# AzureLeon1/DiffSpectra

Hardware: AMD Instinct MI355X
Metric: molecules/sec, 1000-step QM9S all-spectra sampling (partial run) (higher is better)
Workload: dtype f32 (GEMMs as split-fp16 x3 MFMA with fp32 accumulate; fp32-level accuracy, parity gates unchanged)

## Files before the change

diffspectra_amd/csrc/ds_device.h:

```cpp
#pragma once
#include <hip/hip_runtime.h>
#include <stdint.h>

typedef float f32x16 __attribute__((ext_vector_type(16)));
typedef float f32x2 __attribute__((ext_vector_type(2)));
typedef _Float16 h4 __attribute__((ext_vector_type(4)));
typedef _Float16 h8 __attribute__((ext_vector_type(8)));
typedef float f32x4 __attribute__((ext_vector_type(4)));

#define DS_LDP 4

__device__ __forceinline__ float ds_silu(float x) { return __fdividef(x, 1.0f + __expf(-x)); }
__device__ __forceinline__ float ds_tanh(float x) {
  const float e = __builtin_amdgcn_exp2f(x * 2.8853900817779268f);
  return fmaf(-2.0f, __builtin_amdgcn_rcpf(e + 1.0f), 1.0f);
}
__device__ __forceinline__ f32x2 ds_tanh2_prescaled(f32x2 t) {
  f32x2 e;
  e.x = __builtin_amdgcn_exp2f(t.x); e.y = __builtin_amdgcn_exp2f(t.y);
  const f32x2 d = e + 1.0f;
  f32x2 r;
  r.x = __builtin_amdgcn_rcpf(d.x); r.y = __builtin_amdgcn_rcpf(d.y);
  return r * -2.0f + 1.0f;
}
// ... 327 lines not shown
#pragma unroll
  for (int m = 0; m < MT; ++m) {
    xa[m][0] = *reinterpret_cast<const h8*>(xr + m * 32 * ldh);
    xa[m][1] = *reinterpret_cast<const h8*>(xr + m * 32 * ldh + K_tile);
  }
#define DS_MMA_(ACC, WV, XV) ACC = TRANS ? __builtin_amdgcn_mfma_f32_32x32x16_f16(WV, XV, ACC, 0, 0, 0) : __builtin_amdgcn_mfma_f32_32x32x16_f16(XV, WV, ACC, 0, 0, 0)
#pragma unroll
  for (int i = 0; i < NKB; ++i) {
    const int in = i + 1 < NKB ? i + 1 : i;
    h8 xn[MT][2];
#pragma unroll
    for (int m = 0; m < MT; ++m) {
      xn[m][0] = *reinterpret_cast<const h8*>(xr + m * 32 * ldh + in * 16);
      xn[m][1] = *reinterpret_cast<const h8*>(xr + m * 32 * ldh + K_tile + in * 16);
    }
    __builtin_amdgcn_sched_barrier(0);
    const h8 a1 = ringA.w1[i % PF], a2 = ringA.w2[i % PF], b1 = ringB.w1[i % PF], b2 = ringB.w2[i % PF];
#pragma unroll
    for (int m = 0; m < MT; ++m) { DS_MMA_(loA[m], a1, xa[m][1]); DS_MMA_(loB[m], b1, xa[m][1]); }
#pragma unroll
    for (int m = 0; m < MT; ++m) { DS_MMA_(hiA[m], a1, xa[m][0]); DS_MMA_(hiB[m], b1, xa[m][0]); }
#pragma unroll
    for (int m = 0; m < MT; ++m) { DS_MMA_(loA[m], a2, xa[m][0]); DS_MMA_(loB[m], b2, xa[m][0]); }
    if (i + PF < NKB) {
      ringA.w1[i % PF] = wload_h(wsA, 0, kb0 + i + PF); ringA.w2[i % PF] = wload_h(wsA, 1, kb0 + i + PF);
      ringB.w1[i % PF] = wload_h(wsB, 0, kb0 + i + PF); ringB.w2[i % PF] = wload_h(wsB, 1, kb0 + i + PF);
    }
    __builtin_amdgcn_sched_barrier(0);
#pragma unroll
    for (int m = 0; m < MT; ++m) { xa[m][0] = xn[m][0]; xa[m][1] = xn[m][1]; }
  }
#undef DS_MMA_
}
template <int MT, bool TRANS, int NKB, int PF>
__device__ __forceinline__ void wave_mma_h_ring_t2(const _Float16* X, int K_tile, const WStreamH& wsA, const WStreamH& wsB, int kb0,
                                                   f32x16 (&hiA)[MT], f32x16 (&loA)[MT], f32x16 (&hiB)[MT], f32x16 (&loB)[MT], int xkb0 = 0) {
  WRingH<PF> ringA, ringB;
#pragma unroll
  for (int i = 0; i < PF; ++i) {
    ringA.w1[i] = wload_h(wsA, 0, kb0 + i); ringA.w2[i] = wload_h(wsA, 1, kb0 + i);
    ringB.w1[i] = wload_h(wsB, 0, kb0 + i); ringB.w2[i] = wload_h(wsB, 1, kb0 + i);
    __builtin_amdgcn_sched_barrier(0);
  }
  wave_mma_h_deep_t2<MT, TRANS, NKB, PF>(X, K_tile, wsA, wsB, ringA, ringB, kb0, hiA, loA, hiB, loB, xkb0);
}

template <int MT, bool TRANS, int NKB, int PF>
__device__ __forceinline__ void wave_mma_h_ring(const _Float16* X, int K_tile, const float* __restrict__ Wh, int N, int K, int col0,
                                                int kb0, f32x16 (&hi)[MT], f32x16 (&lo)[MT], int xkb0 = 0) {
  const WStreamH ws = wstream_h(Wh, N, K, col0);
  WRingH<PF> ring;
  wring_h<PF>(ring, ws, kb0);
  wave_mma_h_deep<MT, TRANS, NKB, PF>(X, K_tile, ws, ring, kb0, hi, lo, xkb0);
}
template <int MT>
__device__ __forceinline__ void split_finish(f32x16 (&hi)[MT], const f32x16 (&lo)[MT]) {
#pragma unroll
  for (int m = 0; m < MT; ++m)
#pragma unroll
    for (int i = 0; i < 16; ++i) hi[m][i] = fmaf(lo[m][i], 1.0f / 2048.0f, hi[m][i]);
}

template <int MT>
__device__ __forceinline__ void acc_zero(f32x16 (&acc)[MT]) {
#pragma unroll
  for (int m = 0; m < MT; ++m)
#pragma unroll
    for (int i = 0; i < 16; ++i) acc[m][i] = 0.0f;
}

template <int MT, class F>
__device__ __forceinline__ void acc_foreach(const f32x16 (&acc)[MT], int row_base, int col0, F f) {
  const int lane = threadIdx.x & 63, r = lane & 31, hh = lane >> 5;
#pragma unroll
  for (int m = 0; m < MT; ++m)
#pragma unroll
    for (int i = 0; i < 16; ++i) f(row_base + m * 32 + acc_row(i, hh), col0 + r, acc[m][i]);
}

struct RowStore {
  __amdgpu_buffer_rsrc_t rsrc;
  int voff;
};
template <int LD>
__device__ __forceinline__ RowStore row_store(float* dst) {
  const int lane = threadIdx.x & 63;
  const unsigned long long pw = reinterpret_cast<unsigned long long>(dst);
  const unsigned long long pu = (static_cast<unsigned long long>(__builtin_amdgcn_readfirstlane(static_cast<int>(pw >> 32))) << 32) |
                                static_cast<unsigned int>(__builtin_amdgcn_readfirstlane(static_cast<int>(pw)));
  RowStore s;
  s.rsrc = __builtin_amdgcn_make_buffer_rsrc(reinterpret_cast<float*>(pu), 0, 0x7fffffff, 0x00020000);
  s.voff = ((4 * (lane >> 5)) * LD + (lane & 31)) * 4;
  return s;
}
__device__ __forceinline__ void row_put(const RowStore& s, int row_byte_off, float v) {
  __builtin_amdgcn_raw_buffer_store_b32(__float_as_uint(v), s.rsrc, s.voff, row_byte_off, 0);
}
template <int MT, int LD, class F>
__device__ __forceinline__ void acc_store(const f32x16 (&acc)[MT], float* __restrict__ dst, int rows_valid, F f) {
  const int lane = threadIdx.x & 63, r = lane & 31, hh = lane >> 5;
  const RowStore st = row_store<LD>(dst);
  if (rows_valid >= 32 * MT) {
#pragma unroll
    for (int m = 0; m < MT; ++m)
#pragma unroll
      for (int i = 0; i < 16; ++i) row_put(st, (m * 32 + (i & 3) + 8 * (i >> 2)) * LD * 4, f(r, acc[m][i]));
  } else {
#pragma unroll
    for (int m = 0; m < MT; ++m)
#pragma unroll
      for (int i = 0; i < 16; ++i) {
        const int row = m * 32 + (i & 3) + 8 * (i >> 2);
        if (row + 4 * hh < rows_valid) row_put(st, row * LD * 4, f(r, acc[m][i]));
      }
  }
}

template <int MTOT, int MT>
__device__ __forceinline__ BFrag tile_first(const float* __restrict__ Wp, int Npad, int K, int nch) {
  constexpr int RG = MTOT / MT;
  const int wave = threadIdx.x >> 6;
  const int it = wave < nch * RG ? wave : 0;
  return bfrag_load(Wp, Npad, (it / RG) * 32, 0, K >> 3);
}

template <int MTOT, int MT, class G>
__device__ __forceinline__ void tile_gemm_blk(const float* X, int ldx, int K, const float* __restrict__ Wp, int Npad, int nch,
                                              G g, const BFrag* first = nullptr) {
  static_assert(MTOT % MT == 0, "row tiling");
// ... 30 lines not shown
```

diffspectra_amd/csrc/ds_forward.hip:

```cpp
#include <hip/hip_runtime.h>
#include <math.h>
#include <stdint.h>
#include <stdlib.h>

#include <atomic>
#include <mutex>
#include <utility>
#include <vector>

#include "../../include/diffspectra_hip.h"
#include "ds_device.h"
#include "ds_host.h"

#define ADAC DS_ADA_COLS
constexpr int DS_NODE_PF = 8;
constexpr int DS_NODE_PF2 = 4;
constexpr int DS_QKV_PF = 4;
constexpr int DS_TWO_STREAM_MAX_PAIRS = 400000;

#ifdef DS_STAMPS
#define DS_STAMP_INIT()                                                                                 \
  unsigned long long _sa[16] = {0, 0, 0, 0, 0, 0, 0, 0, 0, 0, 0, 0, 0, 0, 0, 0};                        \
  unsigned long long _t0 = __builtin_amdgcn_s_memtime()
#define DS_STAMP(i)                                                                                     \
// ... 6 lines not shown
  do {                                                                                                  \
    asm volatile("s_waitcnt vmcnt(0) lgkmcnt(0)" ::: "memory");                                         \
    DS_STAMP(i);                                                                                        \
  } while (0)
#define DS_STAMP_FLUSH(t)                                                                               \
  do {                                                                                                  \
    if (threadIdx.x == (t))                                                                             \
      for (int _i = 0; _i < 16; ++_i)                                                                   \
        if (_sa[_i]) atomicAdd(reinterpret_cast<unsigned long long*>(c.ws.flags + 16) + _i, _sa[_i]);   \
  } while (0)
#else
#define DS_STAMP_INIT()
#define DS_STAMP(i)
#define DS_STAMP_W(i)
#define DS_STAMP_FLUSH(t)
#endif

namespace {

using dst::clear;
using dst::record;
using dst::wait;

struct Ctx {
  ds_layout L;
  ds_workspace ws;
  const float* wbase;
  const int64_t* woff;
  float edge_th, cutoff;
};

__device__ __forceinline__ const float* BW(const Ctx& c, int blk, int slot) {
  return c.wbase + c.woff[blk * DS_W_BLOCK_SLOTS + slot];
}
__device__ __forceinline__ const float* GW(const Ctx& c, int slot) {
  return c.wbase + c.woff[DS_NBLOCKS * DS_W_BLOCK_SLOTS + slot];
}

__device__ __forceinline__ float rbf_feature(float x, int k, const float* __restrict__ mean, const float* __restrict__ stdv,
                                             const float* __restrict__ astd) {
  if (k == 0) return x;
  const float z = (x - mean[k - 1]) / stdv[k - 1];
  return expf(-0.5f * (z * z)) / astd[k - 1];
}

__global__ void k_time_feat(Ctx c, const float* __restrict__ noise_level) {
  const int b = blockIdx.x * blockDim.x + threadIdx.x;
  if (b >= c.L.B) return;
  const float* w = GW(c, DS_GW_SIN_W);
  const float x = noise_level[b];
  float* f = c.ws.tfeat + (size_t)b * 24;
  f[0] = x;
  for (int i = 0; i < 8; ++i) {
    const float fr = ((x * w[i]) * 2.0f) * 3.14159265358979323846f;
    f[1 + i] = sinf(fr);
    f[9 + i] = cosf(fr);
  }
  for (int i = 17; i < 24; ++i) f[i] = 0.0f;
}

__global__ void k_pair_flags(Ctx c, const float* __restrict__ cond_x, const float* __restrict__ cond_edge_x) {
  const int p = blockIdx.x * blockDim.x + threadIdx.x;
  const bool valid = p < c.L.Pp;
  int bits = 3;
  bool nonzero = false;
  if (valid && cond_x != nullptr) {
// ... 589 lines not shown
  const int Nn = c.L.Nn;
  {
    float4 v[16];
#pragma unroll
    for (int u = 0; u < 16; ++u) {
      const int idx = tid + u * 256, row = idx >> 6, k4 = idx & 63;
      v[u] = reinterpret_cast<const float4*>(c.ws.attn + (size_t)min(row0 + row, Nn - 1) * 256)[k4];
    }
#pragma unroll
    for (int u = 0; u < 16; ++u) {
      const int idx = tid + u * 256, row = idx >> 6, k4 = idx & 63;
      split_store4(&A1[row][0], 256, 4 * k4, row0 + row < Nn ? v[u] : make_float4(0, 0, 0, 0));
    }
  }
  __syncthreads();
  const int mt = wave >> 1, cc = wave & 1;
  if (row0 + mt * 32 >= Nn) return;
  f32x16 acc[1], lo[1];
  acc_zero<1>(acc);
  acc_zero<1>(lo);
  wave_mma_h_ring<1, false, 16, DS_NODE_PF>(&A1[mt * 32][0], 256, BW(c, blk, DS_BW_N2E_H), 64, 256, cc * 32, 0, acc, lo);
  split_finish<1>(acc, lo);
  acc_store<1, 64>(acc, c.ws.u + (size_t)(row0 + mt * 32) * 64 + cc * 32, Nn - row0 - mt * 32, [](int, float v) { return v; });
  (void)lane;
}

template <bool N2E>
__global__ __launch_bounds__(256, 2) void k_node_update(Ctx c, int blk) {
  ds_fp16_saturate();
  constexpr int T = 32, LDH = 2 * 256 + 8;
  __shared__ __attribute__((aligned(16))) _Float16 B1[T][LDH];
  __shared__ __attribute__((aligned(16))) _Float16 H2[T][LDH];
  __shared__ int rmol[T];
  const int tid = threadIdx.x, wave = tid >> 6, row0 = blockIdx.x * T;
  const int Nn = c.L.Nn;
  const float* ada = c.ws.ada;
  if (tid < T) rmol[tid] = (row0 + tid < Nn) ? c.L.node_mol[row0 + tid] : 0;
  __syncthreads();
  {
    const int lane = tid & 63, g = lane >> 4, j = lane & 15;
    float4 va[2][4], vh[2][4], vg[2][4], sh[2][4], sc[2][4];
#pragma unroll
    for (int ps = 0; ps < 2; ++ps) {
      const int row = 8 * wave + 4 * ps + g;
      const size_t gr = (size_t)min(row0 + row, Nn - 1);
      const float4* ad = reinterpret_cast<const float4*>(ada + (size_t)rmol[row] * ADAC + blk * DS_ADA_BLOCK_STRIDE + DS_ADA_NODE) + j;
      const float4* ap = reinterpret_cast<const float4*>(c.ws.attn + gr * 256) + j;
      const float4* hp = reinterpret_cast<const float4*>(c.ws.h + gr * 256) + j;
#pragma unroll
      for (int u = 0; u < 4; ++u) {
        va[ps][u] = ap[16 * u];
        vh[ps][u] = hp[16 * u];
        vg[ps][u] = ad[128 + 16 * u];
        sh[ps][u] = ad[192 + 16 * u];
        sc[ps][u] = ad[256 + 16 * u];
      }
    }
#pragma unroll
    for (int ps = 0; ps < 2; ++ps) {
      const int row = 8 * wave + 4 * ps + g;
      float4 r[4];
#pragma unroll
      for (int u = 0; u < 4; ++u) {
        if (row0 + row >= Nn) va[ps][u] = vh[ps][u] = make_float4(0, 0, 0, 0);
        if (N2E) split_store4(&B1[row][0], 256, 64 * u + 4 * j, va[ps][u]);
        r[u].x = vh[ps][u].x + vg[ps][u].x * va[ps][u].x; r[u].y = vh[ps][u].y + vg[ps][u].y * va[ps][u].y;
        r[u].z = vh[ps][u].z + vg[ps][u].z * va[ps][u].z; r[u].w = vh[ps][u].w + vg[ps][u].w * va[ps][u].w;
      }
      ln_mod_quad256(r, sh[ps], sc[ps]);
#pragma unroll
      for (int u = 0; u < 4; ++u) split_store4(&H2[row][0], 256, 64 * u + 4 * j, r[u]);
    }
  }
  __syncthreads();
  if (N2E) {
    if (wave < 2) {
      f32x16 acc[1], lo[1];
      acc_zero<1>(acc);
      acc_zero<1>(lo);
      wave_mma_h_ring<1, false, 16, DS_NODE_PF>(&B1[0][0], 256, BW(c, blk, DS_BW_N2E_H), 64, 256, wave * 32, 0, acc, lo);
      split_finish<1>(acc, lo);
      acc_store<1, 64>(acc, c.ws.u + (size_t)row0 * 64 + wave * 32, Nn - row0, [](int, float v) { return v; });
    }
    __syncthreads();
  }
  {
    const float* b1 = BW(c, blk, DS_BW_FF1_B);
    const float* W1 = BW(c, blk, DS_BW_FF1_H);
    const float* W2 = BW(c, blk, DS_BW_FF2_H);
    f32x16 acc2[2][1], lo2[2][1];
    acc_zero<1>(acc2[0]); acc_zero<1>(acc2[1]);
    acc_zero<1>(lo2[0]); acc_zero<1>(lo2[1]);
    const int mA = rmol[0], mB = rmol[min(T, Nn - row0) - 1];
    const float* gsec = ada + blk * DS_ADA_BLOCK_STRIDE + DS_ADA_NODE + 1280;
    float gAv[2], gBv[2], bbv[2];
#pragma unroll
    for (int cc = 0; cc < 2; ++cc) {
      const int col = (wave + 4 * cc) * 32 + (tid & 31);
      gAv[cc] = gsec[(size_t)mA * ADAC + col]; gBv[cc] = gsec[(size_t)mB * ADAC + col]; bbv[cc] = BW(c, blk, DS_BW_FF2_B)[col];
    }
    for (int half = 0; half < 2; ++half) {
      {
        asm volatile("" ::: "memory");
        const int hhf = (tid & 63) >> 5;
        f32x16 acc[2][1], lo[2][1];
#pragma unroll
        for (int cc = 0; cc < 2; ++cc) {
          const float bf = b1[half * 256 + (wave + 4 * cc) * 32 + (tid & 31)];
#pragma unroll
          for (int i = 0; i < 16; ++i) acc[cc][0][i] = bf;
          acc_zero<1>(lo[cc]);
        }
        wave_mma_h_ring_t2<1, false, 16, DS_NODE_PF2>(&H2[0][0], 256, wstream_h(W1, 512, 256, (half * 8 + wave) * 32),
                                                     wstream_h(W1, 512, 256, (half * 8 + wave + 4) * 32), 0, acc[0], lo[0], acc[1], lo[1]);
#pragma unroll
        for (int cc = 0; cc < 2; ++cc) {
          split_finish<1>(acc[cc], lo[cc]);
          const int colf = (wave + 4 * cc) * 32 + (tid & 31);
#pragma unroll
          for (int i = 0; i < 16; i += 2) {
            f32x2 v;
            v.x = acc[cc][0][i]; v.y = acc[cc][0][i + 1];
            v = ds_silu2(v);
            const int r0 = acc_row(i, hhf);
            split_store1(&B1[r0][0], 256, colf, v.x);
            split_store1(&B1[r0 + 1][0], 256, colf, v.y);
          }
        }
      }
      __syncthreads();
      asm volatile("" ::: "memory");
      wave_mma_h_ring_t2<1, false, 16, DS_NODE_PF2>(&B1[0][0], 256, wstream_h(W2, 256, 512, wave * 32), wstream_h(W2, 256, 512, (wave + 4) * 32),
                                                   half * 16, acc2[0], lo2[0], acc2[1], lo2[1], half * 16);
      __syncthreads();
    }
    split_finish<1>(acc2[0], lo2[0]);
    split_finish<1>(acc2[1], lo2[1]);
    const int hhl = (tid & 63) >> 5;
    const bool two = mB - mA <= 1;
    bool isB[16];
#pragma unroll
    for (int i = 0; i < 16; ++i) isB[i] = rmol[acc_row(i, hhl)] != mA;
    const int rows_here = Nn - row0;
#pragma unroll
    for (int cc = 0; cc < 2; ++cc) {
      const int col = (wave + 4 * cc) * 32 + (tid & 31);
      const float gA = gAv[cc], gB = gBv[cc], bb = bbv[cc];
      const RowStore st = row_store<256>(c.ws.h + (size_t)row0 * 256 + (wave + 4 * cc) * 32);
#pragma unroll
      for (int i = 0; i < 16; ++i) {
        const int row = acc_row(i, hhl);
        float g = isB[i] ? gB : gA;
        if (!two) { const int m = rmol[row]; if (m != mA && m != mB) g = gsec[(size_t)m * ADAC + col]; }
        const float out = split_load1(&H2[row][0], 256, col) + g * (acc2[cc][0][i] + bb);
        split_store1(&H2[row][0], 256, col, out);
        if (row < rows_here) row_put(st, ((i & 3) + 8 * (i >> 2)) * 256 * 4, out);
      }
    }
  }
  __syncthreads();
  {
    const float* br = BW(c, blk, DS_BW_NODE_RO_B);
    auto ws_of = [&](int it) {
      return it < 2 ? wstream_h(BW(c, blk, DS_BW_NODE_RO_H), 64, 256, it * 32) : wstream_h(BW(c, blk, DS_BW_AC_H), 512, 256, (it - 2) * 32);
    };
    auto bias_of = [&](int it) { return it < 2 ? br[it * 32 + (tid & 31)] : 0.0f; };
    auto store_of = [&](int it, const f32x16 (&acc)[1]) {
      if (it < 2) acc_store<1, 768>(acc, c.ws.atom_hids + (size_t)row0 * 768 + 256 + 64 * blk + it * 32, Nn - row0, [](int, float v) { return v; });
      else acc_store<1, 512>(acc, c.ws.ac + (size_t)row0 * 512 + (it - 2) * 32, Nn - row0, [](int, float v) { return v; });
    };
#pragma unroll
    for (int pr = 0; pr < 2; ++pr) {
      asm volatile("" ::: "memory");
      const int itA = wave + 8 * pr, itB = itA + 4;
      f32x16 acc[2][1], lo[2][1];
      const float bA = bias_of(itA), bB = bias_of(itB);
#pragma unroll
      for (int i = 0; i < 16; ++i) { acc[0][0][i] = bA; acc[1][0][i] = bB; }
      acc_zero<1>(lo[0]); acc_zero<1>(lo[1]);
      wave_mma_h_ring_t2<1, false, 16, DS_NODE_PF2>(&H2[0][0], 256, ws_of(itA), ws_of(itB), 0, acc[0], lo[0], acc[1], lo[1]);
      split_finish<1>(acc[0], lo[0]);
      store_of(itA, acc[0]);
      split_finish<1>(acc[1], lo[1]);
      store_of(itB, acc[1]);
    }
    if (wave < 2) {
      asm volatile("" ::: "memory");
      const int it = 16 + wave;
      f32x16 acc[1], lo[1];
      acc_zero<1>(acc);
      acc_zero<1>(lo);
      wave_mma_h_ring<1, false, 16, DS_NODE_PF>(&H2[0][0], 256, BW(c, blk, DS_BW_AC_H), 512, 256, (it - 2) * 32, 0, acc, lo);
      split_finish<1>(acc, lo);
      store_of(it, acc);
    }
  }
}

__global__ __launch_bounds__(256, 2) void k_edge_update(Ctx c, int blk) {
  ds_fp16_saturate();
  DS_STAMP_INIT();
  constexpr int R = 32, LDW = 64 + DS_LDP;
  __shared__ __attribute__((aligned(16))) float E2s[4][R][LDW];
  __shared__ __attribute__((aligned(16))) float Ds[4][R][LDW];
  __shared__ int idx_s[4][3][R];
  const int tid = threadIdx.x, wave = tid >> 6, lane = tid & 63, hh = lane >> 5, r31 = lane & 31;
  constexpr int LDW2 = 2 * 64 + 8;
  float(*E2)[LDW] = E2s[wave];
  _Float16* E2h = reinterpret_cast<_Float16*>(&E2s[wave][0][0]);
  _Float16* Dh = reinterpret_cast<_Float16*>(&Ds[wave][0][0]);
  int* rmol = idx_s[wave][0];
  int* rpa = idx_s[wave][1];
  int* rpb = idx_s[wave][2];
  const int Pp = c.L.Pp;
  const int row0 = (blockIdx.x * 4 + wave) * R;
  if (row0 >= Pp) return;
  const int valid = min(R, Pp - row0);
  const float* ada = c.ws.ada + blk * DS_ADA_BLOCK_STRIDE + DS_ADA_EDGE;
  if (lane < R) {
    const int p = min(row0 + lane, Pp - 1);
    rmol[lane] = c.L.pair_mol[p]; rpa[lane] = c.L.pair_a[p]; rpb[lane] = c.L.pair_b[p];
  }
  DS_STAMP(0);
  {
    const float4* bn = reinterpret_cast<const float4*>(BW(c, blk, DS_BW_N2E_B));
    float rm[4], rs[4], ra[4];
#pragma unroll
// ... 146 lines not shown
    const float* bd = BW(c, blk, DS_BW_ED_B);
    const float* Wd = BW(c, blk, DS_BW_ED_H);
    float* ed = c.ws.ed + (size_t)row0 * 256;
    for (int ch = 0; ch < 8; ++ch) {
      asm volatile("" ::: "memory");
      f32x16 acc[1], lo[1];
      const float b = bd[ch * 32 + r31];
#pragma unroll
      for (int i = 0; i < 16; ++i) acc[0][i] = b;
      acc_zero<1>(lo);
      wave_mma_h<1>(E2h, 64, Wd, 256, 128, ch * 32, 0, 4, acc, lo);
      wave_mma_h<1>(Dh, 64, Wd, 256, 128, ch * 32, 4, 8, acc, lo, 4);
      split_finish<1>(acc, lo);
      acc_store<1, 256>(acc, ed + ch * 32, valid, [](int, float v) { return v; });
    }
  }
  DS_STAMP(6);
  DS_STAMP_FLUSH(0);
}

constexpr int EQUI_NCW = 4;
constexpr int EQUI_NLW = 4;
__global__ __launch_bounds__((EQUI_NCW + EQUI_NLW) * 64) void k_equi_pairs(Ctx c, int blk) {
  ds_fp16_saturate();
  constexpr int NCW = EQUI_NCW, NLW = EQUI_NLW;
  constexpr int T = 64, TP = 32, LDH = 2 * 256 + 8, NCH = 8;
  constexpr int CPW = NCH / NCW;
  constexpr int PPW = TP / NLW;
  constexpr int NPASS = PPW / 2;
  static_assert(NCH % NCW == 0 && TP % NLW == 0 && PPW % 2 == 0, "role split");
  static_assert(CPW == 2, "a consumer wave runs its two feature chunks against shared X fragments");
  __shared__ __attribute__((aligned(16))) _Float16 Xh[2][T][LDH];
  __shared__ __attribute__((aligned(16))) float part[2][NCH][T][4];
  __shared__ __attribute__((aligned(16))) float dirs[3][T][4];
  __shared__ __attribute__((aligned(16))) float cb0[NCH][2][16];
  __shared__ __attribute__((aligned(16))) float cw2[NCH][2][4][16];
  const int tid = threadIdx.x, wave = tid >> 6, lane = tid & 63, hh = lane >> 5;
  const int Pp = c.L.Pp;
  const int ntiles_all = (Pp + TP - 1) / TP;
  const int tiles_per_wg = (ntiles_all + (int)gridDim.x - 1) / (int)gridDim.x;
  const int ntiles = min(ntiles_all, ((int)blockIdx.x + 1) * tiles_per_wg);
  const float* adq = c.ws.ada + blk * DS_ADA_BLOCK_STRIDE + DS_ADA_EQUI;
  const bool consumer = wave < NCW;
  const float cscale = BW(c, blk, DS_BW_COORD_SCALE)[0];
  DS_STAMP_INIT();
  {
    const float* b0 = BW(c, blk, DS_BW_CM0_B);
    const float* w2 = BW(c, blk, DS_BW_CM2_W);
    for (int idx = tid; idx < NCH * 2 * 16; idx += (NCW + NLW) * 64) {
      const int ch = idx >> 5, h = (idx >> 4) & 1, i = idx & 15, f = ch * 32 + acc_row(i, h);
      cb0[ch][h][i] = b0[f];
#pragma unroll
      for (int o = 0; o < 3; ++o) cw2[ch][h][o][i] = wp_at(w2, 32, f, o);
      cw2[ch][h][3][i] = 0.0f;
    }
  }
  if (consumer) __builtin_amdgcn_s_setprio(0); else __builtin_amdgcn_s_setprio(3);

  const int lw = __builtin_amdgcn_readfirstlane(wave - NCW);

  auto tail = [&](int tile, int pb, int gen) {
    const int p0 = tile * TP;
    const int npairs = min(TP, Pp - p0);
    if ((lane >> 1) < npairs) {
      float4 sacc = reinterpret_cast<const float4*>(&part[pb][0][lane][0])[0];
#pragma unroll
      for (int w = 1; w < NCH; ++w) {
// ... 49 lines not shown
          for (int o = 0; o < 3; ++o) wv[o] = reinterpret_cast<const float4*>(&cw2[ch][hh][o][0])[q4];
#pragma unroll
          for (int m = 0; m < 2; ++m) {
            f32x2 y0, y1;
            y0.x = acc1[m][4 * q4]; y0.y = acc1[m][4 * q4 + 1]; y1.x = acc1[m][4 * q4 + 2]; y1.y = acc1[m][4 * q4 + 3];
            y0 = ds_silu2(y0); y1 = ds_silu2(y1);
#pragma unroll
            for (int o = 0; o < 3; ++o) {
              so[m][o] = __builtin_elementwise_fma(f32x2{wv[o].x, wv[o].y}, y0, so[m][o]);
              so[m][o] = __builtin_elementwise_fma(f32x2{wv[o].z, wv[o].w}, y1, so[m][o]);
            }
          }
        }
        float4 o4;
        float* op = &o4.x;
#pragma unroll
        for (int o = 0; o < 3; ++o) {
          const float s0 = so[0][o].x + so[0][o].y, s1 = so[1][o].x + so[1][o].y;
          const auto sw = __builtin_amdgcn_permlane32_swap(__float_as_uint(s0), __float_as_uint(s1), false, false);
          op[o] = __uint_as_float(sw[0]) + __uint_as_float(sw[1]);
        }
        o4.w = 0.0f;
        reinterpret_cast<float4*>(&part[buf][ch][lane][0])[0] = o4;
      };
      {
        f32x16 accA[2], loA[2], accB[2], loB[2];
        bias_init(wave, accA);
        bias_init(wave + NCW, accB);
        acc_zero<2>(loA);
        acc_zero<2>(loB);
        wave_mma_h_deep_t2<2, true, 16, PF>(&Xh[buf][0][0], 256, wsh[0], wsh[1], ring, ringB, 0, accA, loA, accB, loB);
        wring_h<PF>(ring, wsh[0], 0);
        wring_h<PF>(ringB, wsh[1], 0);
        DS_STAMP(3);
        split_finish<2>(accA, loA);
        epilogue(wave, accA);
        DS_STAMP(10);
        split_finish<2>(accB, loB);
        epilogue(wave + NCW, accB);
        DS_STAMP(11);
      }
      if (wave == 0 && it > 0) tail(tile - stride, buf ^ 1, (it + 2) % 3);
      DS_STAMP(1);
      __syncthreads();
      DS_STAMP(2);
    }
    if (wave == 0) tail(ntiles - 1, (it + 1) & 1, (it + 2) % 3);
    DS_STAMP_FLUSH(0);
  } else {
    const int g = lane >> 4, j = lane & 15, up = g >> 1, gdir = g & 1, slot = (lane >> 1) & (PPW - 1), dir = lane & 1;
    const float4* ac4 = reinterpret_cast<const float4*>(c.ws.ac);
    const float4* ed4 = reinterpret_cast<const float4*>(c.ws.ed);
    int pv_c = 0, av_c = 0, bv_c = 0, mv_c = 0, adj_c = 0;
    int pv_x = 0, av_x = 0, bv_x = 0, mv_x = 0, adj_x = 0;
#define DS_EQUI_FETCH_IDX(TILE, PV, AV, BV, MV, ADJ)                                                   \
    do {                                                                                               \
      const int p0_ = (TILE) * TP, qv_ = lw * PPW + slot;                                              \
      PV = qv_ < min(TP, Pp - p0_) ? p0_ + qv_ : 0;  \
      AV = c.L.pair_a[PV]; BV = c.L.pair_b[PV]; MV = c.L.pair_mol[PV]; ADJ = c.ws.adj[PV];             \
    } while (0)
#define DS_EQUI_ISSUE_B(BT, BVREG)                                                                     \
    do {                                                                                               \
      const int r0_ = __builtin_amdgcn_readlane(BVREG, 4 * (BT)), r1_ = __builtin_amdgcn_readlane(BVREG, 4 * (BT) + 2); \
      const float4* pb_ = ac4 + (size_t)(up ? r1_ : r0_) * 128 + (gdir ? 0 : 64) + j;                  \
      _Pragma("unroll") for (int u = 0; u < 4; ++u) Bv[BT][u] = pb_[16 * u];                           \
    } while (0)
    float4 Bv[NPASS][4], Ka[4], sh[4], sc[4];
    int cur_m = -1, cur_a = -1;
    DS_EQUI_FETCH_IDX(first, pv_c, av_c, bv_c, mv_c, adj_c);
    float4 pr = make_float4(0, 0, 0, 0), pc = pr;
    if (lane < 2 * PPW) {
      pr = reinterpret_cast<const float4*>(c.ws.pos)[dir ? bv_c : av_c];
      pc = reinterpret_cast<const float4*>(c.ws.pos)[dir ? av_c : bv_c];
    }
    if (first + stride < ntiles) DS_EQUI_FETCH_IDX(first + stride, pv_x, av_x, bv_x, mv_x, adj_x);
#pragma unroll
    for (int bt = 0; bt < NPASS; ++bt) DS_EQUI_ISSUE_B(bt, bv_c);
    DS_STAMP(4);
    int k = 0;
    for (int tile = first;; tile += stride, ++k) {
      const bool have = tile < ntiles;
      if (have) {
        const int buf = k & 1, gen = k % 3;
        const int p0 = tile * TP, npairs = min(TP, Pp - p0);
        const bool have_next = tile + stride < ntiles;
        int na[PPW], pm[PPW], pp[PPW];
#pragma unroll
        for (int u = 0; u < PPW; ++u) {
          pp[u] = __builtin_amdgcn_readlane(pv_c, 2 * u); na[u] = __builtin_amdgcn_readlane(av_c, 2 * u);
          pm[u] = __builtin_amdgcn_readlane(mv_c, 2 * u);
        }
#define DS_EQUI_ISSUE_A(BT)                                                                            \
        do {                                                                                           \
          const int ra_ = up ? na[2 * (BT) + 1] : na[2 * (BT)];                                        \
          if (ra_ != cur_a) {                                                                          \
            const float4* pa_ = ac4 + (size_t)ra_ * 128 + (gdir ? 64 : 0) + j;                         \
            _Pragma("unroll") for (int u = 0; u < 4; ++u) Ka[u] = pa_[16 * u];                         \
            cur_a = ra_;                                                                               \
          }                                                                                            \
        } while (0)
#define DS_EQUI_ISSUE_M(BT)                                                                            \
        do {                                                                                           \
          const int m_ = up ? pm[2 * (BT) + 1] : pm[2 * (BT)];                                         \
          if (m_ != cur_m) {                                                                           \
            const float4* ps_ = reinterpret_cast<const float4*>(adq + (size_t)m_ * ADAC) + j;          \
            _Pragma("unroll") for (int u = 0; u < 4; ++u) { sh[u] = ps_[16 * u]; sc[u] = ps_[64 + 16 * u]; }  \
            cur_m = m_;                                                                                \
          }                                                                                            \
        } while (0)
        DS_EQUI_ISSUE_A(0);
        DS_EQUI_ISSUE_M(0);
#pragma unroll
        for (int i = 0; i < PPW; ++i)
          __builtin_amdgcn_global_load_lds((const __attribute__((address_space(1))) void*)(ed4 + (size_t)pp[i] * 64 + lane),
                                           (__attribute__((address_space(3))) void*)&Xh[buf][2 * (lw * PPW + i)][0], 16, 0, 0);
        __builtin_amdgcn_sched_barrier(0);
        DS_STAMP(5);
        if (lane < 2 * PPW) {
          const float dx = pr.x - pc.x, dy = pr.y - pc.y, dz = pr.z - pc.z;
          const float nrm = fmaxf(__builtin_amdgcn_sqrtf(dx * dx + dy * dy + dz * dz), 1e-8f);
          const float sn = cscale * __builtin_amdgcn_rcpf(nrm);
          float4 d;
          d.x = dx * sn; d.y = dy * sn; d.z = dz * sn; d.w = __int_as_float(adj_c);
          reinterpret_cast<float4*>(&dirs[gen][2 * (lw * PPW + slot) + dir][0])[0] = d;
          if (have_next) {
            pr = reinterpret_cast<const float4*>(c.ws.pos)[dir ? bv_x : av_x];
            pc = reinterpret_cast<const float4*>(c.ws.pos)[dir ? av_x : bv_x];
          }
        }
        DS_STAMP(6);
        asm volatile("s_waitcnt vmcnt(0)" ::: "memory");
        __builtin_amdgcn_sched_barrier(0);
        DS_STAMP(8);
#pragma unroll
        for (int bt = 0; bt < NPASS; ++bt) {
          const int q = lw * PPW + 2 * bt + up;
          float4 x[4];
#pragma unroll
          for (int u = 0; u < 4; ++u) {
            const float4 e = reinterpret_cast<const float4*>(&Xh[buf][2 * q][0])[16 * u + j];
            x[u].x = (Ka[u].x + Bv[bt][u].x) + e.x; x[u].y = (Ka[u].y + Bv[bt][u].y) + e.y;
            x[u].z = (Ka[u].z + Bv[bt][u].z) + e.z; x[u].w = (Ka[u].w + Bv[bt][u].w) + e.w;
          }
          __builtin_amdgcn_sched_barrier(0);
          if (have_next) DS_EQUI_ISSUE_B(bt, bv_x);
          if (bt + 1 < NPASS) DS_EQUI_ISSUE_A(bt + 1);
          __builtin_amdgcn_sched_barrier(0);
          DS_STAMP(12);
          ln_mod_quad256(x, sh, sc);
          _Float16* xr = &Xh[buf][2 * q + gdir][0];
#pragma unroll
          for (int u = 0; u < 4; ++u) split_store4(xr, 256, 64 * u + 4 * j, x[u]);
          if (bt + 1 < NPASS) DS_EQUI_ISSUE_M(bt + 1);
          DS_STAMP(14);
        }
        if (npairs < TP) {
          for (int i = 0; i < PPW; ++i) {
            const int qz = lw * PPW + i;
            if (qz >= npairs) {
              float4* z = reinterpret_cast<float4*>(&Xh[buf][2 * qz][0]);
              z[lane] = make_float4(0, 0, 0, 0);
              z[64 + lane] = make_float4(0, 0, 0, 0);
              if (lane < 2) z[128 + lane] = make_float4(0, 0, 0, 0);
            }
          }
        }
      }
      DS_STAMP(7);
      __syncthreads();
      DS_STAMP(9);
      if (!have) break;
      pv_c = pv_x; av_c = av_x; bv_c = bv_x; mv_c = mv_x; adj_c = adj_x;
      if (tile + 2 * stride < ntiles) DS_EQUI_FETCH_IDX(tile + 2 * stride, pv_x, av_x, bv_x, mv_x, adj_x);
    }
#undef DS_EQUI_FETCH_IDX
#undef DS_EQUI_ISSUE_B
#undef DS_EQUI_ISSUE_A
#undef DS_EQUI_ISSUE_M
    DS_STAMP_FLUSH(NCW * 64);
  }
}

__global__ __launch_bounds__(64) void k_pos_update(Ctx c, int last) {
  const int m = blockIdx.x, r = threadIdx.x;
  const int n0 = c.L.node_off[m], n = c.L.node_off[m + 1] - n0;
  const int p0 = c.L.pair_off[m];
  if (n <= 0) return;
  float x = 0.0f, y = 0.0f, z = 0.0f;
  if (r < n) {
    const float4* tr = reinterpret_cast<const float4*>(c.ws.tr);
    float sx = 0.0f, sy = 0.0f, sz = 0.0f;
    for (int c0 = 0; c0 < n; c0 += 8) {
      float4 t[8];
#pragma unroll
      for (int u = 0; u < 8; ++u) {
        const int cc = c0 + u;
        t[u] = make_float4(0, 0, 0, 0);
        if (cc < n && cc != r) {
          const int lo = r < cc ? r : cc, hi = r < cc ? cc : r;
          const int pl = lo * (2 * n - lo - 1) / 2 + (hi - lo - 1);
          t[u] = tr[(size_t)(p0 + pl) * 2 + (r < cc ? 0 : 1)];
        }
      }
#pragma unroll
      for (int u = 0; u < 8; ++u)
        if (c0 + u < n && c0 + u != r) { sx += t[u].x; sy += t[u].y; sz += t[u].z; }
    }
    const float* pp = c.ws.pos + (size_t)(n0 + r) * 4;
    x = pp[0] + sx; y = pp[1] + sy; z = pp[2] + sz;
  }
  const float fn = (float)n;
// ... 464 lines not shown
```

Before: 236.9.

## Prefetch next GEMM weight rings before stores/barriers in node update kernel

Restructures the node-update kernel so each GEMM's weight prefetch ring is filled before the preceding stores and __syncthreads complete, overlapping global weight loads with epilogue stores. Weight pointers are made wave-uniform via readfirstlane and hoisted, and biases are preloaded. Boundary stores switch to buffer-resource clamped stores instead of per-row predicates. The molecule gating adds a three-molecule fast path, which removes scattered loads. The cost is higher register pressure from holding the rings across phases.

```diff
diff --git a/diffspectra_amd/csrc/ds_device.h b/diffspectra_amd/csrc/ds_device.h
--- a/diffspectra_amd/csrc/ds_device.h
+++ b/diffspectra_amd/csrc/ds_device.h
@@ -383,16 +383,20 @@
   }
 #undef DS_MMA_
 }
+template <int PF>
+__device__ __forceinline__ void wring_h_t2(WRingH<PF>& ringA, WRingH<PF>& ringB, const WStreamH& wsA, const WStreamH& wsB, int kb0) {
+#pragma unroll
+  for (int i = 0; i < PF; ++i) {
+    ringA.w1[i] = wload_h(wsA, 0, kb0 + i); ringA.w2[i] = wload_h(wsA, 1, kb0 + i);
+    ringB.w1[i] = wload_h(wsB, 0, kb0 + i); ringB.w2[i] = wload_h(wsB, 1, kb0 + i);
+    __builtin_amdgcn_sched_barrier(0);
+  }
+}
 template <int MT, bool TRANS, int NKB, int PF>
 __device__ __forceinline__ void wave_mma_h_ring_t2(const _Float16* X, int K_tile, const WStreamH& wsA, const WStreamH& wsB, int kb0,
                                                    f32x16 (&hiA)[MT], f32x16 (&loA)[MT], f32x16 (&hiB)[MT], f32x16 (&loB)[MT], int xkb0 = 0) {
   WRingH<PF> ringA, ringB;
-#pragma unroll
-  for (int i = 0; i < PF; ++i) {
-    ringA.w1[i] = wload_h(wsA, 0, kb0 + i); ringA.w2[i] = wload_h(wsA, 1, kb0 + i);
-    ringB.w1[i] = wload_h(wsB, 0, kb0 + i); ringB.w2[i] = wload_h(wsB, 1, kb0 + i);
-    __builtin_amdgcn_sched_barrier(0);
-  }
+  wring_h_t2<PF>(ringA, ringB, wsA, wsB, kb0);
   wave_mma_h_deep_t2<MT, TRANS, NKB, PF>(X, K_tile, wsA, wsB, ringA, ringB, kb0, hiA, loA, hiB, loB, xkb0);
 }
 
@@ -446,6 +450,28 @@
 }
 __device__ __forceinline__ void row_put(const RowStore& s, int row_byte_off, float v) {
   __builtin_amdgcn_raw_buffer_store_b32(__float_as_uint(v), s.rsrc, s.voff, row_byte_off, 0);
+}
+template <int LD>
+__device__ __forceinline__ RowStore row_store_clamped(float* dst, int rows_valid) {
+  const int lane = threadIdx.x & 63;
+  const unsigned long long pw = reinterpret_cast<unsigned long long>(dst);
+  const unsigned long long pu = (static_cast<unsigned long long>(__builtin_amdgcn_readfirstlane(static_cast<int>(pw >> 32))) << 32) |
+                                static_cast<unsigned int>(__builtin_amdgcn_readfirstlane(static_cast<int>(pw)));
+  RowStore s;
+  s.rsrc = __builtin_amdgcn_make_buffer_rsrc(reinterpret_cast<float*>(pu), 0, __builtin_amdgcn_readfirstlane(min(rows_valid, 1 << 16)) * LD * 4, 0x00020000);
+  s.voff = ((4 * (lane >> 5)) * LD + (lane & 31)) * 4;
+  return s;
+}
+__device__ __forceinline__ void row_put_clamped(const RowStore& s, int row_byte_off, float v) {
+  __builtin_amdgcn_raw_buffer_store_b32(__float_as_uint(v), s.rsrc, s.voff + row_byte_off, 0, 0);
+}
+template <int MT, int LD>
+__device__ __forceinline__ void acc_store_clamped(const f32x16 (&acc)[MT], float* __restrict__ dst, int rows_valid) {
+  const RowStore st = row_store_clamped<LD>(dst, min(rows_valid, 32 * MT));
+#pragma unroll
+  for (int m = 0; m < MT; ++m)
+#pragma unroll
+    for (int i = 0; i < 16; ++i) row_put_clamped(st, (m * 32 + (i & 3) + 8 * (i >> 2)) * LD * 4, acc[m][i]);
 }
 template <int MT, int LD, class F>
 __device__ __forceinline__ void acc_store(const f32x16 (&acc)[MT], float* __restrict__ dst, int rows_valid, F f) {
diff --git a/diffspectra_amd/csrc/ds_forward.hip b/diffspectra_amd/csrc/ds_forward.hip
--- a/diffspectra_amd/csrc/ds_forward.hip
+++ b/diffspectra_amd/csrc/ds_forward.hip
@@ -62,6 +62,11 @@
 
 __device__ __forceinline__ const float* BW(const Ctx& c, int blk, int slot) {
   return c.wbase + c.woff[blk * DS_W_BLOCK_SLOTS + slot];
+}
+__device__ __forceinline__ const float* BWU(const Ctx& c, int blk, int slot) {
+  const int64_t o = c.woff[blk * DS_W_BLOCK_SLOTS + slot];
+  return c.wbase + ((static_cast<int64_t>(__builtin_amdgcn_readfirstlane(static_cast<int>(o >> 32))) << 32) |
+                    static_cast<unsigned int>(__builtin_amdgcn_readfirstlane(static_cast<int>(o))));
 }
 __device__ __forceinline__ const float* GW(const Ctx& c, int slot) {
   return c.wbase + c.woff[DS_NBLOCKS * DS_W_BLOCK_SLOTS + slot];
@@ -717,9 +722,16 @@
   __shared__ __attribute__((aligned(16))) _Float16 B1[T][LDH];
   __shared__ __attribute__((aligned(16))) _Float16 H2[T][LDH];
   __shared__ int rmol[T];
-  const int tid = threadIdx.x, wave = tid >> 6, row0 = blockIdx.x * T;
+  const int tid = threadIdx.x, wave = __builtin_amdgcn_readfirstlane(tid >> 6), row0 = blockIdx.x * T;
   const int Nn = c.L.Nn;
   const float* ada = c.ws.ada;
+  const float* const b1 = BWU(c, blk, DS_BW_FF1_B);
+  const float* const W1 = BWU(c, blk, DS_BW_FF1_H);
+  const float* const W2 = BWU(c, blk, DS_BW_FF2_H);
+  const float* const b2 = BWU(c, blk, DS_BW_FF2_B);
+  const float* const br = BWU(c, blk, DS_BW_NODE_RO_B);
+  const float* const Wro = BWU(c, blk, DS_BW_NODE_RO_H);
+  const float* const Wac = BWU(c, blk, DS_BW_AC_H);
   if (tid < T) rmol[tid] = (row0 + tid < Nn) ? c.L.node_mol[row0 + tid] : 0;
   __syncthreads();
   {
@@ -758,31 +770,34 @@
     }
   }
   __syncthreads();
-  if (N2E) {
-    if (wave < 2) {
-      f32x16 acc[1], lo[1];
-      acc_zero<1>(acc);
-      acc_zero<1>(lo);
-      wave_mma_h_ring<1, false, 16, DS_NODE_PF>(&B1[0][0], 256, BW(c, blk, DS_BW_N2E_H), 64, 256, wave * 32, 0, acc, lo);
-      split_finish<1>(acc, lo);
-      acc_store<1, 64>(acc, c.ws.u + (size_t)row0 * 64 + wave * 32, Nn - row0, [](int, float v) { return v; });
-    }
-    __syncthreads();
-  }
-  {
-    const float* b1 = BW(c, blk, DS_BW_FF1_B);
-    const float* W1 = BW(c, blk, DS_BW_FF1_H);
-    const float* W2 = BW(c, blk, DS_BW_FF2_H);
+  f32x16 accu[1];
+  if (N2E && wave < 2) {
+    f32x16 lo[1];
+    acc_zero<1>(accu);
+    acc_zero<1>(lo);
+    wave_mma_h_ring<1, false, 16, DS_NODE_PF>(&B1[0][0], 256, BWU(c, blk, DS_BW_N2E_H), 64, 256, wave * 32, 0, accu, lo);
+    split_finish<1>(accu, lo);
+  }
+  WRingH<DS_NODE_PF2> ringA, ringB;
+  const auto ws1_of = [&](int half, int cc) { return wstream_h(W1, 512, 256, (half * 8 + wave + 4 * cc) * 32); };
+  {
     f32x16 acc2[2][1], lo2[2][1];
     acc_zero<1>(acc2[0]); acc_zero<1>(acc2[1]);
     acc_zero<1>(lo2[0]); acc_zero<1>(lo2[1]);
     const int mA = rmol[0], mB = rmol[min(T, Nn - row0) - 1];
+    const int mM = min(mA + 1, mB);
     const float* gsec = ada + blk * DS_ADA_BLOCK_STRIDE + DS_ADA_NODE + 1280;
-    float gAv[2], gBv[2], bbv[2];
+    float gAv[2], gMv[2], gBv[2], bbv[2], bfv[2][2];
 #pragma unroll
     for (int cc = 0; cc < 2; ++cc) {
       const int col = (wave + 4 * cc) * 32 + (tid & 31);
-      gAv[cc] = gsec[(size_t)mA * ADAC + col]; gBv[cc] = gsec[(size_t)mB * ADAC + col]; bbv[cc] = BW(c, blk, DS_BW_FF2_B)[col];
+      gAv[cc] = gsec[(size_t)mA * ADAC + col]; gMv[cc] = gsec[(size_t)mM * ADAC + col]; gBv[cc] = gsec[(size_t)mB * ADAC + col];
+      bbv[cc] = b2[col]; bfv[0][cc] = b1[col]; bfv[1][cc] = b1[256 + col];
+    }
+    wring_h_t2<DS_NODE_PF2>(ringA, ringB, ws1_of(0, 0), ws1_of(0, 1), 0);
+    if (N2E) {
+      if (wave < 2) acc_store_clamped<1, 64>(accu, c.ws.u + (size_t)row0 * 64 + wave * 32, Nn - row0);
+      __syncthreads();
     }
     for (int half = 0; half < 2; ++half) {
       {
@@ -791,13 +806,13 @@
         f32x16 acc[2][1], lo[2][1];
 #pragma unroll
         for (int cc = 0; cc < 2; ++cc) {
-          const float bf = b1[half * 256 + (wave + 4 * cc) * 32 + (tid & 31)];
+          const float bf = half ? bfv[1][cc] : bfv[0][cc];
 #pragma unroll
           for (int i = 0; i < 16; ++i) acc[cc][0][i] = bf;
           acc_zero<1>(lo[cc]);
         }
-        wave_mma_h_ring_t2<1, false, 16, DS_NODE_PF2>(&H2[0][0], 256, wstream_h(W1, 512, 256, (half * 8 + wave) * 32),
-                                                     wstream_h(W1, 512, 256, (half * 8 + wave + 4) * 32), 0, acc[0], lo[0], acc[1], lo[1]);
+        if (half) wring_h_t2<DS_NODE_PF2>(ringA, ringB, ws1_of(1, 0), ws1_of(1, 1), 0);
+        wave_mma_h_deep_t2<1, false, 16, DS_NODE_PF2>(&H2[0][0], 256, ws1_of(half, 0), ws1_of(half, 1), ringA, ringB, 0, acc[0], lo[0], acc[1], lo[1]);
 #pragma unroll
         for (int cc = 0; cc < 2; ++cc) {
           split_finish<1>(acc[cc], lo[cc]);
@@ -822,62 +837,70 @@
     split_finish<1>(acc2[0], lo2[0]);
     split_finish<1>(acc2[1], lo2[1]);
     const int hhl = (tid & 63) >> 5;
-    const bool two = mB - mA <= 1;
-    bool isB[16];
-#pragma unroll
-    for (int i = 0; i < 16; ++i) isB[i] = rmol[acc_row(i, hhl)] != mA;
-    const int rows_here = Nn - row0;
+    const bool three = mB - mA <= 2;
+    bool isA[16], isB[16];
+#pragma unroll
+    for (int i = 0; i < 16; ++i) {
+      const int m = rmol[acc_row(i, hhl)];
+      isA[i] = m == mA; isB[i] = m == mB;
+    }
 #pragma unroll
     for (int cc = 0; cc < 2; ++cc) {
       const int col = (wave + 4 * cc) * 32 + (tid & 31);
-      const float gA = gAv[cc], gB = gBv[cc], bb = bbv[cc];
-      const RowStore st = row_store<256>(c.ws.h + (size_t)row0 * 256 + (wave + 4 * cc) * 32);
+      const float gA = gAv[cc], gM = gMv[cc], gB = gBv[cc], bb = bbv[cc];
+      float gv[16];
+      if (three) {
+#pragma unroll
+        for (int i = 0; i < 16; ++i) gv[i] = isA[i] ? gA : (isB[i] ? gB : gM);
+      } else {
+#pragma unroll
+        for (int i = 0; i < 16; ++i) gv[i] = gsec[(size_t)rmol[acc_row(i, hhl)] * ADAC + col];
+      }
 #pragma unroll
       for (int i = 0; i < 16; ++i) {
         const int row = acc_row(i, hhl);
-        float g = isB[i] ? gB : gA;
-        if (!two) { const int m = rmol[row]; if (m != mA && m != mB) g = gsec[(size_t)m * ADAC + col]; }
-        const float out = split_load1(&H2[row][0], 256, col) + g * (acc2[cc][0][i] + bb);
-        split_store1(&H2[row][0], 256, col, out);
-        if (row < rows_here) row_put(st, ((i & 3) + 8 * (i >> 2)) * 256 * 4, out);
-      }
-    }
-  }
-  __syncthreads();
-  {
-    const float* br = BW(c, blk, DS_BW_NODE_RO_B);
-    auto ws_of = [&](int it) {
-      return it < 2 ? wstream_h(BW(c, blk, DS_BW_NODE_RO_H), 64, 256, it * 32) : wstream_h(BW(c, blk, DS_BW_AC_H), 512, 256, (it - 2) * 32);
+        acc2[cc][0][i] = split_load1(&H2[row][0], 256, col) + gv[i] * (acc2[cc][0][i] + bb);
+        split_store1(&H2[row][0], 256, col, acc2[cc][0][i]);
+      }
+    }
+    auto ws_of = [&](int it) { return it < 2 ? wstream_h(Wro, 64, 256, it * 32) : wstream_h(Wac, 512, 256, (it - 2) * 32); };
+    auto store_of = [&](int it, const f32x16 (&acc)[1]) {
+      if (it < 2) acc_store_clamped<1, 768>(acc, c.ws.atom_hids + (size_t)row0 * 768 + 256 + 64 * blk + it * 32, Nn - row0);
+      else acc_store_clamped<1, 512>(acc, c.ws.ac + (size_t)row0 * 512 + (it - 2) * 32, Nn - row0);
     };
-    auto bias_of = [&](int it) { return it < 2 ? br[it * 32 + (tid & 31)] : 0.0f; };
-    auto store_of = [&](int it, const f32x16 (&acc)[1]) {
-      if (it < 2) acc_store<1, 768>(acc, c.ws.atom_hids + (size_t)row0 * 768 + 256 + 64 * blk + it * 32, Nn - row0, [](int, float v) { return v; });
-      else acc_store<1, 512>(acc, c.ws.ac + (size_t)row0 * 512 + (it - 2) * 32, Nn - row0, [](int, float v) { return v; });
-    };
+    const float bro = br[min(wave, 1) * 32 + (tid & 31)];
+    wring_h_t2<DS_NODE_PF2>(ringA, ringB, ws_of(wave), ws_of(wave + 4), 0);
+#pragma unroll
+    for (int cc = 0; cc < 2; ++cc)
+      acc_store_clamped<1, 256>(acc2[cc], c.ws.h + (size_t)row0 * 256 + (wave + 4 * cc) * 32, Nn - row0);
+    __syncthreads();
+    WRingH<DS_NODE_PF> ring1;
+    const auto ws_last = wstream_h(Wac, 512, 256, (14 + min(wave, 1)) * 32);
 #pragma unroll
     for (int pr = 0; pr < 2; ++pr) {
       asm volatile("" ::: "memory");
       const int itA = wave + 8 * pr, itB = itA + 4;
       f32x16 acc[2][1], lo[2][1];
-      const float bA = bias_of(itA), bB = bias_of(itB);
-#pragma unroll
-      for (int i = 0; i < 16; ++i) { acc[0][0][i] = bA; acc[1][0][i] = bB; }
+      const float bA = pr == 0 && wave < 2 ? bro : 0.0f;
+#pragma unroll
+      for (int i = 0; i < 16; ++i) { acc[0][0][i] = bA; acc[1][0][i] = 0.0f; }
       acc_zero<1>(lo[0]); acc_zero<1>(lo[1]);
-      wave_mma_h_ring_t2<1, false, 16, DS_NODE_PF2>(&H2[0][0], 256, ws_of(itA), ws_of(itB), 0, acc[0], lo[0], acc[1], lo[1]);
+      wave_mma_h_deep_t2<1, false, 16, DS_NODE_PF2>(&H2[0][0], 256, ws_of(itA), ws_of(itB), ringA, ringB, 0, acc[0], lo[0], acc[1], lo[1]);
       split_finish<1>(acc[0], lo[0]);
+      split_finish<1>(acc[1], lo[1]);
+      if (pr == 0) wring_h_t2<DS_NODE_PF2>(ringA, ringB, ws_of(wave + 8), ws_of(wave + 12), 0);
+      else if (wave < 2) wring_h<DS_NODE_PF>(ring1, ws_last, 0);
       store_of(itA, acc[0]);
-      split_finish<1>(acc[1], lo[1]);
       store_of(itB, acc[1]);
     }
     if (wave < 2) {
       asm volatile("" ::: "memory");
-      const int it = 16 + wave;
       f32x16 acc[1], lo[1];
       acc_zero<1>(acc);
       acc_zero<1>(lo);
-      wave_mma_h_ring<1, false, 16, DS_NODE_PF>(&H2[0][0], 256, BW(c, blk, DS_BW_AC_H), 512, 256, (it - 2) * 32, 0, acc, lo);
+      wave_mma_h_deep<1, false, 16, DS_NODE_PF>(&H2[0][0], 256, ws_last, ring1, 0, acc, lo);
       split_finish<1>(acc, lo);
-      store_of(it, acc);
+      store_of(16 + wave, acc);
     }
   }
 }
```

Result: no change. 238.6, median of 6 (+0.7%).

## Prefetch edge rows into registers and move consumer barrier before epilogue

Applied to the files above, without the earlier changes.

The producer (LN) waves now load edge features into registers one tile ahead, alongside the A/B node-feature prefetch, instead of doing global_load_lds followed by a full vmcnt(0) wait. Index fetching is pipelined two tiles deep and the A-row reload cache check is dropped. The consumer waves move their block barrier to just after the MMA split-finish, ahead of the epilogue, and grow the dirs buffer to four generations so the epilogue and tail can overlap the producers' next tile. This should hide global memory latency in the producer waves, at the cost of more registers and some redundant loads past the last tile.

```diff
diff --git a/diffspectra_amd/csrc/ds_forward.hip b/diffspectra_amd/csrc/ds_forward.hip
--- a/diffspectra_amd/csrc/ds_forward.hip
+++ b/diffspectra_amd/csrc/ds_forward.hip
@@ -1090,7 +1090,7 @@
   static_assert(CPW == 2, "a consumer wave runs its two feature chunks against shared X fragments");
   __shared__ __attribute__((aligned(16))) _Float16 Xh[2][T][LDH];
   __shared__ __attribute__((aligned(16))) float part[2][NCH][T][4];
-  __shared__ __attribute__((aligned(16))) float dirs[3][T][4];
+  __shared__ __attribute__((aligned(16))) float dirs[4][T][4];
   __shared__ __attribute__((aligned(16))) float cb0[NCH][2][16];
   __shared__ __attribute__((aligned(16))) float cw2[NCH][2][4][16];
   const int tid = threadIdx.x, wave = tid >> 6, lane = tid & 63, hh = lane >> 5;
@@ -1206,20 +1206,23 @@
         wave_mma_h_deep_t2<2, true, 16, PF>(&Xh[buf][0][0], 256, wsh[0], wsh[1], ring, ringB, 0, accA, loA, accB, loB);
         wring_h<PF>(ring, wsh[0], 0);
         wring_h<PF>(ringB, wsh[1], 0);
+        split_finish<2>(accA, loA);
+        split_finish<2>(accB, loB);
         DS_STAMP(3);
-        split_finish<2>(accA, loA);
+        __syncthreads();
+        DS_STAMP(2);
         epilogue(wave, accA);
         DS_STAMP(10);
-        split_finish<2>(accB, loB);
         epilogue(wave + NCW, accB);
         DS_STAMP(11);
       }
-      if (wave == 0 && it > 0) tail(tile - stride, buf ^ 1, (it + 2) % 3);
+      if (wave == 0 && it > 0) tail(tile - stride, buf ^ 1, (it + 3) & 3);
       DS_STAMP(1);
-      __syncthreads();
-      DS_STAMP(2);
-    }
-    if (wave == 0) tail(ntiles - 1, (it + 1) & 1, (it + 2) % 3);
+    }
+    __syncthreads();
+    DS_STAMP(2);
+    if (wave == 0) tail(ntiles - 1, (it + 1) & 1, (it + 3) & 3);
+    DS_STAMP(1);
     DS_STAMP_FLUSH(0);
   } else {
     const int g = lane >> 4, j = lane & 15, up = g >> 1, gdir = g & 1, slot = (lane >> 1) & (PPW - 1), dir = lane & 1;
@@ -1227,6 +1230,7 @@
     const float4* ed4 = reinterpret_cast<const float4*>(c.ws.ed);
     int pv_c = 0, av_c = 0, bv_c = 0, mv_c = 0, adj_c = 0;
     int pv_x = 0, av_x = 0, bv_x = 0, mv_x = 0, adj_x = 0;
+    int pv_n = 0, av_n = 0, bv_n = 0, mv_n = 0, adj_n = 0;
 #define DS_EQUI_FETCH_IDX(TILE, PV, AV, BV, MV, ADJ)                                                   \
     do {                                                                                               \
       const int p0_ = (TILE) * TP, qv_ = lw * PPW + slot;                                              \
@@ -1239,55 +1243,54 @@
       const float4* pb_ = ac4 + (size_t)(up ? r1_ : r0_) * 128 + (gdir ? 0 : 64) + j;                  \
       _Pragma("unroll") for (int u = 0; u < 4; ++u) Bv[BT][u] = pb_[16 * u];                           \
     } while (0)
-    float4 Bv[NPASS][4], Ka[4], sh[4], sc[4];
-    int cur_m = -1, cur_a = -1;
+#define DS_EQUI_ISSUE_E(BT, PVREG)                                                                     \
+    do {                                                                                               \
+      const int e0_ = __builtin_amdgcn_readlane(PVREG, 4 * (BT)), e1_ = __builtin_amdgcn_readlane(PVREG, 4 * (BT) + 2); \
+      const float4* pe_ = ed4 + (size_t)(up ? e1_ : e0_) * 64 + j;                                     \
+      _Pragma("unroll") for (int u = 0; u < 4; ++u) Ev[BT][u] = pe_[16 * u];                           \
+    } while (0)
+#define DS_EQUI_ISSUE_A(A0, A1)                                                                        \
+    do {                                                                                               \
+      const float4* pa_ = ac4 + (size_t)(up ? (A1) : (A0)) * 128 + (gdir ? 64 : 0) + j;                \
+      _Pragma("unroll") for (int u = 0; u < 4; ++u) Ka[u] = pa_[16 * u];                               \
+    } while (0)
+#define DS_EQUI_ISSUE_M(M0, M1)                                                                        \
+    do {                                                                                               \
+      const int m_ = up ? (M1) : (M0);                                                                 \
+      if (m_ != cur_m) {                                                                               \
+        const float4* ps_ = reinterpret_cast<const float4*>(adq + (size_t)m_ * ADAC) + j;              \
+        _Pragma("unroll") for (int u = 0; u < 4; ++u) { sh[u] = ps_[16 * u]; sc[u] = ps_[64 + 16 * u]; }  \
+        cur_m = m_;                                                                                    \
+      }                                                                                                \
+    } while (0)
+    float4 Bv[NPASS][4], Ev[NPASS][4], Ka[4], sh[4], sc[4];
+    int cur_m = -1;
     DS_EQUI_FETCH_IDX(first, pv_c, av_c, bv_c, mv_c, adj_c);
     float4 pr = make_float4(0, 0, 0, 0), pc = pr;
     if (lane < 2 * PPW) {
       pr = reinterpret_cast<const float4*>(c.ws.pos)[dir ? bv_c : av_c];
       pc = reinterpret_cast<const float4*>(c.ws.pos)[dir ? av_c : bv_c];
     }
-    if (first + stride < ntiles) DS_EQUI_FETCH_IDX(first + stride, pv_x, av_x, bv_x, mv_x, adj_x);
+    DS_EQUI_FETCH_IDX(first + stride, pv_x, av_x, bv_x, mv_x, adj_x);
 #pragma unroll
     for (int bt = 0; bt < NPASS; ++bt) DS_EQUI_ISSUE_B(bt, bv_c);
+#pragma unroll
+    for (int bt = 0; bt < NPASS; ++bt) DS_EQUI_ISSUE_E(bt, pv_c);
+    DS_EQUI_ISSUE_A(__builtin_amdgcn_readlane(av_c, 0), __builtin_amdgcn_readlane(av_c, 2));
+    DS_EQUI_ISSUE_M(__builtin_amdgcn_readlane(mv_c, 0), __builtin_amdgcn_readlane(mv_c, 2));
     DS_STAMP(4);
     int k = 0;
     for (int tile = first;; tile += stride, ++k) {
       const bool have = tile < ntiles;
       if (have) {
-        const int buf = k & 1, gen = k % 3;
+        const int buf = k & 1, gen = k & 3;
         const int p0 = tile * TP, npairs = min(TP, Pp - p0);
-        const bool have_next = tile + stride < ntiles;
-        int na[PPW], pm[PPW], pp[PPW];
+        int na[PPW], pm[PPW];
 #pragma unroll
         for (int u = 0; u < PPW; ++u) {
-          pp[u] = __builtin_amdgcn_readlane(pv_c, 2 * u); na[u] = __builtin_amdgcn_readlane(av_c, 2 * u);
-          pm[u] = __builtin_amdgcn_readlane(mv_c, 2 * u);
+          na[u] = __builtin_amdgcn_readlane(av_c, 2 * u); pm[u] = __builtin_amdgcn_readlane(mv_c, 2 * u);
         }
-#define DS_EQUI_ISSUE_A(BT)                                                                            \
-        do {                                                                                           \
-          const int ra_ = up ? na[2 * (BT) + 1] : na[2 * (BT)];                                        \
-          if (ra_ != cur_a) {                                                                          \
-            const float4* pa_ = ac4 + (size_t)ra_ * 128 + (gdir ? 64 : 0) + j;                         \
-            _Pragma("unroll") for (int u = 0; u < 4; ++u) Ka[u] = pa_[16 * u];                         \
-            cur_a = ra_;                                                                               \
-          }                                                                                            \
-        } while (0)
-#define DS_EQUI_ISSUE_M(BT)                                                                            \
-        do {                                                                                           \
-          const int m_ = up ? pm[2 * (BT) + 1] : pm[2 * (BT)];                                         \
-          if (m_ != cur_m) {                                                                           \
-            const float4* ps_ = reinterpret_cast<const float4*>(adq + (size_t)m_ * ADAC) + j;          \
-            _Pragma("unroll") for (int u = 0; u < 4; ++u) { sh[u] = ps_[16 * u]; sc[u] = ps_[64 + 16 * u]; }  \
-            cur_m = m_;                                                                                \
-          }                                                                                            \
-        } while (0)
-        DS_EQUI_ISSUE_A(0);
-        DS_EQUI_ISSUE_M(0);
-#pragma unroll
-        for (int i = 0; i < PPW; ++i)
-          __builtin_amdgcn_global_load_lds((const __attribute__((address_space(1))) void*)(ed4 + (size_t)pp[i] * 64 + lane),
-                                           (__attribute__((address_space(3))) void*)&Xh[buf][2 * (lw * PPW + i)][0], 16, 0, 0);
+        DS_EQUI_FETCH_IDX(tile + 2 * stride, pv_n, av_n, bv_n, mv_n, adj_n);
         __builtin_amdgcn_sched_barrier(0);
         DS_STAMP(5);
         if (lane < 2 * PPW) {
@@ -1297,35 +1300,33 @@
           float4 d;
           d.x = dx * sn; d.y = dy * sn; d.z = dz * sn; d.w = __int_as_float(adj_c);
           reinterpret_cast<float4*>(&dirs[gen][2 * (lw * PPW + slot) + dir][0])[0] = d;
-          if (have_next) {
-            pr = reinterpret_cast<const float4*>(c.ws.pos)[dir ? bv_x : av_x];
-            pc = reinterpret_cast<const float4*>(c.ws.pos)[dir ? av_x : bv_x];
-          }
+          pr = reinterpret_cast<const float4*>(c.ws.pos)[dir ? bv_x : av_x];
+          pc = reinterpret_cast<const float4*>(c.ws.pos)[dir ? av_x : bv_x];
         }
         DS_STAMP(6);
-        asm volatile("s_waitcnt vmcnt(0)" ::: "memory");
-        __builtin_amdgcn_sched_barrier(0);
-        DS_STAMP(8);
 #pragma unroll
         for (int bt = 0; bt < NPASS; ++bt) {
           const int q = lw * PPW + 2 * bt + up;
           float4 x[4];
 #pragma unroll
           for (int u = 0; u < 4; ++u) {
-            const float4 e = reinterpret_cast<const float4*>(&Xh[buf][2 * q][0])[16 * u + j];
+            const float4 e = Ev[bt][u];
             x[u].x = (Ka[u].x + Bv[bt][u].x) + e.x; x[u].y = (Ka[u].y + Bv[bt][u].y) + e.y;
             x[u].z = (Ka[u].z + Bv[bt][u].z) + e.z; x[u].w = (Ka[u].w + Bv[bt][u].w) + e.w;
           }
           __builtin_amdgcn_sched_barrier(0);
-          if (have_next) DS_EQUI_ISSUE_B(bt, bv_x);
-          if (bt + 1 < NPASS) DS_EQUI_ISSUE_A(bt + 1);
+          if (bt + 1 < NPASS) DS_EQUI_ISSUE_A(na[2 * bt + 2], na[2 * bt + 3]);
+          else DS_EQUI_ISSUE_A(__builtin_amdgcn_readlane(av_x, 0), __builtin_amdgcn_readlane(av_x, 2));
+          DS_EQUI_ISSUE_B(bt, bv_x);
+          DS_EQUI_ISSUE_E(bt, pv_x);
           __builtin_amdgcn_sched_barrier(0);
           DS_STAMP(12);
           ln_mod_quad256(x, sh, sc);
           _Float16* xr = &Xh[buf][2 * q + gdir][0];
 #pragma unroll
           for (int u = 0; u < 4; ++u) split_store4(xr, 256, 64 * u + 4 * j, x[u]);
-          if (bt + 1 < NPASS) DS_EQUI_ISSUE_M(bt + 1);
+          if (bt + 1 < NPASS) DS_EQUI_ISSUE_M(pm[2 * bt + 2], pm[2 * bt + 3]);
+          else DS_EQUI_ISSUE_M(__builtin_amdgcn_readlane(mv_x, 0), __builtin_amdgcn_readlane(mv_x, 2));
           DS_STAMP(14);
         }
         if (npairs < TP) {
@@ -1345,12 +1346,15 @@
       DS_STAMP(9);
       if (!have) break;
       pv_c = pv_x; av_c = av_x; bv_c = bv_x; mv_c = mv_x; adj_c = adj_x;
-      if (tile + 2 * stride < ntiles) DS_EQUI_FETCH_IDX(tile + 2 * stride, pv_x, av_x, bv_x, mv_x, adj_x);
+      pv_x = pv_n; av_x = av_n; bv_x = bv_n; mv_x = mv_n; adj_x = adj_n;
     }
 #undef DS_EQUI_FETCH_IDX
 #undef DS_EQUI_ISSUE_B
+#undef DS_EQUI_ISSUE_E
 #undef DS_EQUI_ISSUE_A
 #undef DS_EQUI_ISSUE_M
+    __syncthreads();
+    DS_STAMP(9);
     DS_STAMP_FLUSH(NCW * 64);
   }
 }
```

Result: no change. 239.3 before, 241.0 after (median of 6 runs) (+0.7%).
